# Zhangwenyao1/DreamVLA

Hardware: AMD Instinct MI355X
Metric: train samples/sec (CALVIN ABC->D, seq_len=7) (higher is better)
Workload: dtype bf16; 1 GPU; DreamVLA CALVIN finetune step, head set C (obs_pred+depth_pred+sam_feat_pred+use_dit_head), B=32/GPU, S=7, window 10, 2x224^2 views, 77 text tokens, hidden 1024 / 24 layers / 16 heads, dropout 0.1 on, AdamW + clip 0.1; global_batch=32, seq_len=7, parallelism=dp1, grad_exchange=GradBucketReducer (flat bf16 buckets, async all-reduce), optimizer=FlatAdamW (HIP: dvla_sumsq_bf16 + dvla_adamw_bf16 on flat buffers)

## Files before the change

dreamvla_amd/_lib.py:

```python
import ctypes as C
import os

_HERE = os.path.dirname(os.path.abspath(__file__))
LIB_PATH = os.environ.get("DVLA_LIB") or os.path.join(_HERE, "libdvla_hip.so")

DT_BF16, DT_F32 = 0, 1
CROP_OUT_U8, CROP_OUT_BF16 = 0, 1
ABI_VERSION = 8
ACT = {"none": 0, "gelu": 1, "gelu_erf": 1, "gelu_tanh": 2, "gelu_new": 2, "relu": 3, "silu": 4,
       "quick_gelu": 5, "tanh": 6, "sigmoid": 7}

DVLA_ERRORS = {-1: "invalid argument", -2: "kernel launch failed", -3: "unsupported shape/alignment"}


class DvlaError(RuntimeError):
    pass


class GemmParams(C.Structure):
    _fields_ = [
        ("A", C.c_void_p), ("lda", C.c_int64), ("a_trans", C.c_int32),
        ("B", C.c_void_p), ("ldb", C.c_int64), ("b_trans", C.c_int32),
        ("C", C.c_void_p), ("ldc", C.c_int64), ("c_dtype", C.c_int32),
        ("M", C.c_int64), ("N", C.c_int64), ("K", C.c_int64),
        ("bias", C.c_void_p), ("bias_dtype", C.c_int32),
        ("act", C.c_int32),
        ("preact", C.c_void_p), ("ld_preact", C.c_int64),
        ("dact_aux", C.c_void_p), ("ld_dact", C.c_int64), ("dact", C.c_int32),
        ("dropout_p", C.c_float), ("seed_lo", C.c_uint32), ("seed_hi", C.c_uint32),
        ("residual", C.c_void_p), ("ld_res", C.c_int64), ("res_rows", C.c_int64),
        ("accumulate", C.c_int32),
        ("split_k", C.c_int32), ("workspace", C.c_void_p),
        ("ksum", C.c_void_p), ("ksum_dtype", C.c_int32), ("ksum_operand", C.c_int32), ("ksum_workspace", C.c_void_p),
        ("a_layernorm", C.c_int32), ("a_ln_eps", C.c_float),
    ]


class AttnParams(C.Structure):
    _fields_ = [
        ("q", C.c_void_p), ("k", C.c_void_p), ("v", C.c_void_p), ("o", C.c_void_p),
        ("q_stride_b", C.c_int64), ("q_stride_t", C.c_int64), ("q_stride_h", C.c_int64),
        ("k_stride_b", C.c_int64), ("k_stride_t", C.c_int64), ("k_stride_h", C.c_int64),
        ("v_stride_b", C.c_int64), ("v_stride_t", C.c_int64), ("v_stride_h", C.c_int64),
        ("o_stride_b", C.c_int64), ("o_stride_t", C.c_int64), ("o_stride_h", C.c_int64),
        ("B", C.c_int32), ("H", C.c_int32), ("Lq", C.c_int32), ("Lk", C.c_int32),
        ("scale", C.c_float),
        ("key_index", C.c_void_p), ("mask_bits_q", C.c_void_p), ("mask_bits_k", C.c_void_p),
        ("tile_map", C.c_void_p),
        ("dropout_p", C.c_float), ("seed_lo", C.c_uint32), ("seed_hi", C.c_uint32),
        ("lse", C.c_void_p),
        ("dout", C.c_void_p), ("do_stride_b", C.c_int64), ("do_stride_t", C.c_int64), ("do_stride_h", C.c_int64),
        ("delta", C.c_void_p),
        ("dq", C.c_void_p), ("dk", C.c_void_p), ("dv", C.c_void_p),
        ("dq_stride_b", C.c_int64), ("dq_stride_t", C.c_int64), ("dq_stride_h", C.c_int64),
        ("dk_stride_b", C.c_int64), ("dk_stride_t", C.c_int64), ("dk_stride_h", C.c_int64),
        ("dv_stride_b", C.c_int64), ("dv_stride_t", C.c_int64), ("dv_stride_h", C.c_int64),
    ]


class MaskRule(C.Structure):
    _fields_ = [("K", C.c_int32), ("num_A", C.c_int32), ("num_B", C.c_int32), ("num_obs", C.c_int32),
                ("action_pred_steps", C.c_int32), ("atten_goal", C.c_int32), ("atten_goal_state", C.c_int32),
                ("atten_only_obs", C.c_int32), ("attn_robot_proprio_state", C.c_int32), ("n_drop", C.c_int32)]


class TokenSrc(C.Structure):
    _fields_ = [("base", C.c_void_p), ("stride_b", C.c_int64), ("stride_s", C.c_int64), ("tok_begin", C.c_int32),
                ("tok_count", C.c_int32)]


class DitSampleParams(C.Structure):
    _fields_ = [("blocks", C.c_void_p),
                ("xemb_w", C.c_void_p), ("xemb_b", C.c_void_p), ("final_w", C.c_void_p), ("final_b", C.c_void_p),
                ("pos", C.c_void_p), ("cond", C.c_void_p),
                ("coef", C.c_void_p), ("noise", C.c_void_p), ("out", C.c_void_p),
                ("workspace", C.c_void_p), ("workspace_bytes", C.c_int64),
                ("cfg_scale", C.c_float), ("ln_eps", C.c_float),
                ("depth", C.c_int32), ("hidden", C.c_int32), ("heads", C.c_int32), ("channels", C.c_int32),
                ("tokens", C.c_int32), ("bs", C.c_int32), ("steps", C.c_int32), ("reserved", C.c_int32)]


class FrameView(C.Structure):
    _fields_ = [("base", C.c_void_p), ("stride_b", C.c_int64), ("stride_t", C.c_int64), ("T", C.c_int32)]


class MaeLossParams(C.Structure):
    _fields_ = [("pred", C.c_void_p), ("pred_stride_n", C.c_int64), ("pred_stride_r", C.c_int64), ("row0", C.c_int32),
                ("patch", C.c_int32),
                ("imgs", C.c_void_p), ("imgs_dtype", C.c_int32), ("norm_pix", C.c_int32), ("H", C.c_int32), ("W", C.c_int32),
                ("mask", C.c_void_p), ("N", C.c_int64)]


_P, _I64, _I32, _F, _U32 = C.c_void_p, C.c_int64, C.c_int32, C.c_float, C.c_uint32
SYMBOLS = {
    "dvla_abi_version": (C.c_int, []),
    "dvla_gemm_bf16": (C.c_int, [C.POINTER(GemmParams), _P]),
    "dvla_gemm_ksum_partial_rows": (C.c_int64, [C.c_int32]),
    "dvla_set_gemm_variant": (None, [C.c_int]),
    "dvla_last_gemm_variant": (C.c_int, []),
    "dvla_set_gemm_schedule": (None, [C.c_int, C.c_int]),
    "dvla_get_gemm_schedule": (None, [C.POINTER(C.c_int), C.POINTER(C.c_int)]),
    "dvla_layernorm_fwd": (C.c_int, [_P, _P, _P, _I32, _P, _P, _P, _I64, _I64, _F, _P]),
    "dvla_layernorm_bwd": (C.c_int, [_P, _P, _P, _I32, _P, _P, _P, _P, _P, _P, _I64, _I64, _P]),
    "dvla_layernorm_bwd_add": (C.c_int, [_P, _P, _P, _I32, _P, _P, _P, _P, _P, _P, _I32, _P, _I64, _I64, _P]),
    "dvla_layernorm_bwd_partial_rows": (_I64, []),
    "dvla_layernorm_fwd_rows": (C.c_int, [_P, _P, _P, _I32, _P, _P, _P, _I64, _I64, _F, _I32, _I32, _I32, _I32, _P]),
    "dvla_layernorm_bwd_rows": (C.c_int, [_P, _P, _P, _I32, _P, _P, _P, _P, _P, _I32, _P, _I64, _I64, _I32, _I32, _I32, _I32, _P]),
    "dvla_attn_fwd": (C.c_int, [C.POINTER(AttnParams), _P]),
    "dvla_attn_bwd": (C.c_int, [C.POINTER(AttnParams), _P]),
    "dvla_attn_small_fwd": (C.c_int, [C.POINTER(AttnParams), _I32, _P]),
    "dvla_attn_small_bwd": (C.c_int, [C.POINTER(AttnParams), _I32, _P]),
    "dvla_attn_hd_fwd": (C.c_int, [C.POINTER(AttnParams), _I32, _P]),
    "dvla_attn_hd_bwd": (C.c_int, [C.POINTER(AttnParams), _I32, _P]),
    "dvla_colsum": (C.c_int, [_P, _I64, _I64, _I64, _P, _P, _P]),
    "dvla_colsum_dt": (C.c_int, [_P, _I64, _I64, _I64, _P, _I32, _P, _P]),
    "dvla_colsum_partial_rows": (_I64, []),
    "dvla_dropout": (C.c_int, [_P, _P, _I64, _I64, _F, _U32, _U32, _P]),
    "dvla_act_bwd": (C.c_int, [_P, _P, _P, _I64, _I64, _I32, _F, _U32, _U32, _P]),
    "dvla_act_bwd_colsum": (C.c_int, [_P, _P, _P, _I64, _I64, _I32, _F, _U32, _U32, _P, _I32, _P, _P]),
    "dvla_act_fwd": (C.c_int, [_P, _P, _I64, _I32, _P]),
    "dvla_ddim_cfg_step": (C.c_int, [_P, _I64, _P, _P, _I64, _I64, _F, _F, _F, _F, _F, _P]),
    "dvla_fm_cfg_step": (C.c_int, [_P, _I64, _P, _P, _I64, _I64, _F, _F, _P]),
    "dvla_dit_sample_workspace_bytes": (C.c_int64, [_I32]),
    "dvla_dit_sample": (C.c_int, [C.POINTER(DitSampleParams), _P]),
    "dvla_dit_sample_fm": (C.c_int, [C.POINTER(DitSampleParams), _P]),
    "dvla_dit_sample_set_stamps": (None, [_P]),
    "dvla_dit_sample_inject_timeouts": (None, [_I32]),
    "dvla_cast_f32_to_bf16": (C.c_int, [_P, _P, _I64, _P]),
    "dvla_cast_bf16_to_f32": (C.c_int, [_P, _P, _I64, _P]),
    "dvla_add": (C.c_int, [_P, _P, _P, _I64, _I64, _P]),
    "dvla_assemble_tokens": (C.c_int, [C.POINTER(TokenSrc), _I32, _P, _I64, _P, _I32, _I32, _I32, _I32, _P]),
    "dvla_mask_tables": (C.c_int, [C.POINTER(MaskRule), _P, _P, _P, _P, _P, _P]),
    "dvla_image_preprocess": (C.c_int, [_P, _P, _P, _I64, _I32, _I32, _I32, C.POINTER(C.c_float), C.POINTER(C.c_float), _P]),
    "dvla_image_resize_u8": (C.c_int, [_P, _P, _I64, _I32, _I32, _I32, _I32, _P, _P, _I32, _P, _P, _I32, _I32, _I32, _I32, _P]),
    "dvla_image_resized_crop": (C.c_int, [_P, _P, _P, _P, _I64, _I32, _I32, _I32, _I32, _I32, _I32, _I32, C.POINTER(C.c_float),
                                          C.POINTER(C.c_float), _P]),
    "dvla_depth_preprocess": (C.c_int, [_P, _P, _P, _I64, _I32, _I32, _I32, _I32, _I32, _I32, _P]),
    "dvla_gather_positions": (C.c_int, [_P, _P, _P, _I32, _I32, _I32, _I32, _I32, _I32, _P]),
    "dvla_dream_render": (C.c_int, [_P, _P, _P, _I64, _I32, _I32, _I32, _I32, C.POINTER(C.c_float), C.POINTER(C.c_float), _P]),
    "dvla_image_quality_partial_len": (C.c_int64, [_I64, _I32, _I32]),
    "dvla_image_quality": (C.c_int, [_P, _P, _I64, _I32, _I32, _P, _P, _P, _P]),
    "dvla_depth_quality_partial_len": (C.c_int64, [_I64, _I32, _I32]),
    "dvla_depth_quality": (C.c_int, [_P, _P, _I64, _I32, _I32, _P, _P, _P, _P]),
    "dvla_loss_partial_len": (C.c_int64, []),
    "dvla_patch_mse_fwd": (C.c_int, [C.POINTER(FrameView), C.POINTER(FrameView), _P, _I64, _P, _P, _P]),
    "dvla_patch_mse_bwd": (C.c_int, [C.POINTER(FrameView), C.POINTER(FrameView), _P, _I64, _P, C.POINTER(FrameView), _P]),
# ... 68 lines not shown
```

dreamvla_amd/csrc/attention.hip:

```cpp
#include "common.h"
#include "../../include/dvla.h"

namespace {

constexpr int AT_THREADS = 256;
constexpr int RM72 = 72;
constexpr int RM_BYTES = 32 * RM72 * 2;
constexpr int PI_BYTES = 16 * 64 * 4;
constexpr float LOG2E = 1.4426950408889634f;
constexpr float LN2 = 0.6931471805599453f;

struct AttnKArgs {
  const bf16_t *q, *k, *v; bf16_t* o;
  int64_t qsb, qst, qsh, ksb, kst, ksh, vsb, vst, vsh, osb, ost, osh;
  int B, H, Lq, Lk;
  float scale;
  const int32_t* key_index;
  const uint32_t *bits_q, *bits_k;
  const uint8_t* tile_map; int nqt, nkt;
  int has_drop; uint32_t drop_thr; float inv_keep; uint32_t seed_lo, seed_hi;
  float c1;
  float* lse;
  const bf16_t* dout; int64_t dsb, dst, dsh;
  float* delta;
// ... 1467 lines not shown
        const float alpha = fast_exp2(m_run - m_safe);
        float rs = 0.f;
#pragma unroll
        for (int rr = 0; rr < 16; ++rr) { sv[rr] = fast_exp2(fmaf(sv[rr], scale_log2, -m_safe)); rs += sv[rr]; }
        rs += __shfl_xor(rs, 32, 64);
        l_run = l_run * alpha + rs;
        m_run = m_new;
        if (__any(alpha != 1.0f)) {
#pragma unroll
          for (int rr = 0; rr < 16; ++rr) { oacc[0][rr] *= alpha; oacc[1][rr] *= alpha; }
        }
        bf16x8 vt4[4];
#pragma unroll
        for (int i = 0; i < 4; ++i) vt4[i] = fa_frag_tr(vs, i >> 1, i & 1, lane);
        __builtin_amdgcn_sched_barrier(0);
        const bf16x8 pf0 = pack_frag(sv), pf1 = pack_frag(sv + 8);
        fa_group4(vt4);
        oacc[0] = __builtin_amdgcn_mfma_f32_32x32x16_bf16(vt4[0], pf0, oacc[0], 0, 0, 0);
        oacc[1] = __builtin_amdgcn_mfma_f32_32x32x16_bf16(vt4[2], pf0, oacc[1], 0, 0, 0);
        oacc[0] = __builtin_amdgcn_mfma_f32_32x32x16_bf16(vt4[1], pf1, oacc[0], 0, 0, 0);
        oacc[1] = __builtin_amdgcn_mfma_f32_32x32x16_bf16(vt4[3], pf1, oacc[1], 0, 0, 0);
      }
      if (q_ok) {
        const float inv_l = l_run > 0.f ? 1.0f / l_run : 0.f;
        store_token(p.o + (int64_t)b * p.osb + (int64_t)q * p.ost + (int64_t)h * p.osh, oacc, inv_l, g, (p.st16 & 1) != 0);
        if (p.lse && g == 0) p.lse[(b * p.H + h) * L + q] = l_run > 0.f ? (m_run + log2f(l_run)) * LN2 : INFINITY;
      }
    }
    __syncthreads();
  }
}


}

static bool attn_span32(int64_t rows, int64_t stride_elems, bool gathered) {
  const int64_t r = gathered ? (rows > (1 << 18) ? rows : (1 << 18)) : rows;
  return stride_elems >= 0 && r * stride_elems * 2 + 128 < (1LL << 32);
}

static bool attn_force_staged() {
  static int v = -1;
  if (v < 0) { const char* e = getenv("DVLA_ATTN_STAGED"); v = (e && e[0] == '1') ? 1 : 0; }
  return v == 1;
}

static bool attn_short_enabled() { const char* e = getenv("DVLA_ATTN_SHORT"); return !(e && e[0] == '0'); }
static bool attn_short_fwd_enabled() { const char* e = getenv("DVLA_ATTN_SHORT_FWD"); return !(e && e[0] == '0'); }
static int attn_num_cus() {
  static int cus = 0;
  if (cus == 0) {
    int dev = 0; hipDeviceProp_t prop;
    cus = (hipGetDevice(&dev) == hipSuccess && hipGetDeviceProperties(&prop, dev) == hipSuccess) ? prop.multiProcessorCount : 256;
  }
  return cus;
}

#ifdef DVLA_ATTN_ABLATION
static int attn_dbg() { const char* e = getenv("DVLA_ATTN_DBG"); return e ? atoi(e) : 0; }
#endif

static dim3 ring_items_grid(int nblk, const AttnKArgs& a) {
  static int forced = -1, cus = 0;
  if (forced < 0) {
    const char* e = getenv("DVLA_ATTN_ITEMS"); forced = e ? atoi(e) : 0;
    int dev = 0; hipDeviceProp_t prop;
// ... 100 lines not shown
  const dim3 grid_dq((unsigned)((a.nqt + 3) / 4), (unsigned)a.H, (unsigned)a.B);
  const dim3 grid_dkv((unsigned)((a.nkt + 3) / 4), (unsigned)a.H, (unsigned)a.B);
  const bool span_kv = attn_span32(a.Lk, a.kst, a.key_index != nullptr) && attn_span32(a.Lk, a.vst, a.key_index != nullptr);
  const bool span_q = attn_span32(a.Lq, a.qst, false) && attn_span32(a.Lq, a.dst, false);
  const bool dq_ring = smem_dq <= 64 * 1024 && span_kv && !attn_force_staged();
  a.fuse_delta = dq_ring ? 1 : 0;
  if (!dq_ring) {
    hipLaunchKernelGGL(attn_delta_kernel, dim3((unsigned)((nrows * 8 + 255) / 256)), dim3(256), 0, stream, a);
    rc = dvla_check_launch();
    if (rc != DVLA_OK) return rc;
  }
  if (dq_ring)
    hipLaunchKernelGGL(attn_bwd_dq_ring_kernel, grid_dq, block, smem_dq, stream, a);
  else
    hipLaunchKernelGGL(attn_bwd_dq_kernel, grid_dq, block, 0, stream, a);
  rc = dvla_check_launch();
  if (rc != DVLA_OK) return rc;
  if (smem_dkv <= 80 * 1024 && span_q && !attn_force_staged()) {
    if (smem_dkv > 64 * 1024) {
      static uint64_t attr_done = 0;
      int dev = 0;
      if (hipGetDevice(&dev) != hipSuccess || dev < 0 || dev >= 64) dev = 0;
      if (!(attr_done & (1ull << dev))) {
        (void)hipFuncSetAttribute(reinterpret_cast<const void*>(attn_bwd_dkv_ring_kernel), hipFuncAttributeMaxDynamicSharedMemorySize, 80 * 1024);
        attr_done |= 1ull << dev;
      }
    }
    hipLaunchKernelGGL(attn_bwd_dkv_ring_kernel, grid_dkv, block, smem_dkv, stream, a);
  }
  else
    hipLaunchKernelGGL(attn_bwd_dkv_kernel, grid_dkv, block, 0, stream, a);
  return dvla_check_launch();
}
```

dreamvla_amd/nn.py:

```python
import torch
from torch import nn

from . import ops


class Linear(nn.Linear):

    def forward(self, x, act="none", residual=None, dropout_p=0.0, ln_eps=None):
        if ln_eps is not None:
            return ops.linear_ln(x, self.weight, self.bias, eps=ln_eps, act=act, residual=residual)
        return ops.linear(x, self.weight, self.bias, act=act, residual=residual, dropout_p=dropout_p)


class LayerNorm(nn.LayerNorm):
    def forward(self, x):
        return ops.layer_norm(x, self.weight, self.bias, self.eps)

    def fork(self, x):
        return ops.layer_norm_fork(x, self.weight, self.bias, self.eps)

    def last_tokens(self, x, keep):
        return ops.layer_norm_last_tokens(x, self.weight, self.bias, self.eps, keep)


# ... 36 lines not shown
        self.head_dim = dim // num_heads
        self.scale = self.head_dim ** -0.5
        self.qkv = Linear(dim, dim * 3, bias=qkv_bias)
        self.proj = Linear(dim, dim)

    def forward(self, x, residual=None, ln_eps=None):
        qkv = self.qkv(x, ln_eps=ln_eps)
        o = ops.self_attention(qkv, self.num_heads, scale=self.scale, head_dim=self.head_dim)
        return self.proj(o, residual=residual)


class Block(nn.Module):

    def __init__(self, dim, num_heads, mlp_ratio=4.0, qkv_bias=False, norm_layer=None, act="gelu_erf"):
        super().__init__()
        norm_layer = norm_layer or LayerNorm
        self.norm1 = norm_layer(dim)
        self.attn = Attention(dim, num_heads=num_heads, qkv_bias=qkv_bias)
        self.norm2 = norm_layer(dim)
        self.mlp = Mlp(in_features=dim, hidden_features=int(dim * mlp_ratio), act=act)

    def forward(self, x):
        if isinstance(self.norm1, LayerNorm) and isinstance(self.norm2, LayerNorm):
            r, n = self.norm1.fork(x)
            x = self.attn(n, residual=r)
            r, n = self.norm2.fork(x)
            return self.mlp(n, residual=r)
        x = self.attn(self.norm1(x), residual=x)
        x = self.mlp(self.norm2(x), residual=x)
        return x

    def forward_shared_suffix(self, prefix, suffix, n_seq):
        x = ops.concat_shared_suffix(prefix, suffix)
        qkv = ops.concat_shared_suffix(self.attn.qkv(self.norm1(prefix)), self.attn.qkv(self.norm1(suffix)))
        o = ops.self_attention(qkv, self.attn.num_heads, scale=self.attn.scale, head_dim=self.attn.head_dim)
        x = self.attn.proj(o, residual=x)
        r, n = self.norm2.fork(x)
        return self.mlp(n, residual=r)


class PatchEmbed(nn.Module):

    def __init__(self, img_size=224, patch_size=16, in_chans=3, embed_dim=768):
        super().__init__()
        self.img_size = (img_size, img_size)
        self.patch_size = (patch_size, patch_size)
        self.grid_size = (img_size // patch_size, img_size // patch_size)
        self.num_patches = self.grid_size[0] * self.grid_size[1]
        self.proj = nn.Conv2d(in_chans, embed_dim, kernel_size=patch_size, stride=patch_size)

    def forward(self, x, pos=None):
        n, c, hh, ww = x.shape
        p = self.patch_size[0]
        gh, gw = hh // p, ww // p
        cols = x.view(n, c, gh, p, gw, p).permute(0, 2, 4, 1, 3, 5).reshape(n * gh * gw, c * p * p)
        w = self.proj.weight.view(self.proj.weight.shape[0], -1)
        y = ops.linear(cols, w, self.proj.bias, residual=pos, res_rows=(gh * gw if pos is not None else 0))
        return y.view(n, gh * gw, -1)
```

dreamvla_amd/ops.py:

```python
import ctypes as C
import math
import os

import torch

from . import _lib
from ._lib import ACT, AttnParams, DT_BF16, DT_F32, GemmParams, check

BF16 = torch.bfloat16


def _stream():
    return torch.cuda.current_stream().cuda_stream


def _req(t, name, dtype=BF16):
    if not isinstance(t, torch.Tensor):
        raise TypeError(f"{name}: expected a tensor")
    if not t.is_cuda:
        raise _lib.DvlaError(f"{name}: tensor is on {t.device}; the DreamVLA HIP path has no CPU fallback")
    if dtype is not None and t.dtype != dtype:
        raise TypeError(f"{name}: expected {dtype}, got {t.dtype} (the kernels compute in bf16; fp32 parameters / activations "
                        f"are accepted by the module-level operators -- linear, mlp, layer_norm, attention -- which keep "
                        f"fp32 masters and run on bf16 shadows)")
# ... 1407 lines not shown
    def forward(ctx, prefix, suffix):
        lib = _lib.load()
        _req(prefix, "concat_shared_suffix.prefix"); _req(suffix, "concat_shared_suffix.suffix")
        n, nq, D = prefix.shape
        ns = suffix.shape[0]
        if suffix.shape[1] != D or D % 8 != 0:
            raise ValueError("concat_shared_suffix: (n, nq, D) and (ns, D) with D % 8 == 0")
        if not (prefix.stride(2) == 1 and prefix.stride(1) == D and prefix.stride(0) % 8 == 0 and prefix.data_ptr() % 16 == 0):
            prefix = prefix.contiguous()
        suffix = suffix.contiguous()
        srcs = (_lib.TokenSrc * 2)()
        srcs[0] = _lib.TokenSrc(prefix.data_ptr(), prefix.stride(0), 0, 0, nq)
        srcs[1] = _lib.TokenSrc(suffix.data_ptr(), 0, 0, nq, ns)
        out = torch.empty((n, nq + ns, D), dtype=BF16, device=prefix.device)
        check(lib.dvla_assemble_tokens(srcs, 2, None, D, out.data_ptr(), n, 1, nq + ns, D, _stream()), "dvla_assemble_tokens")
        ctx.nq, ctx.ns = nq, ns
        return out

    @staticmethod
    def backward(ctx, g):
        g = _req(g, "concat_shared_suffix.grad").contiguous()
        n, L, D = g.shape
        dp = g[:, :ctx.nq] if ctx.needs_input_grad[0] else None
        ds = None
        if ctx.needs_input_grad[1]:
            ds = colsum(g.view(n, L * D)[:, ctx.nq * D:], out_dtype=BF16).view(ctx.ns, D)
        return dp, ds


def concat_shared_suffix(prefix, suffix):
    return _ConcatSharedSuffix.apply(to_compute(prefix), to_compute(suffix))


def assemble_tokens(parts, pos=None):
    if len(parts) > 16:
        raise ValueError("assemble_tokens: at most 16 parts")
    return _AssembleTokens.apply(to_compute(pos), *[to_compute(t) for t in parts])


class _Dropout(torch.autograd.Function):
    @staticmethod
    def forward(ctx, x, p):
        _req(x, "dropout.input")
        seed = next_seed()
        ctx.p, ctx.seed, ctx.shape = p, seed, x.shape
        return dropout_raw(x.reshape(-1, x.shape[-1]), p, seed).view(x.shape)

    @staticmethod
    def backward(ctx, dy):
        return dropout_raw(dy.reshape(-1, ctx.shape[-1]), ctx.p, ctx.seed).view(ctx.shape), None


def dropout(x, p, training):
    if not training or p <= 0.0:
        return x
    return _Dropout.apply(to_compute(x), float(p))


class _Act(torch.autograd.Function):
    @staticmethod
    def forward(ctx, x, act):
        _req(x, "act.input")
        ctx.act = act
        if ctx.needs_input_grad[0]:
            ctx.save_for_backward(x)
        return act_fwd_raw(x, act)
# ... 300 lines not shown
```

include/dvla.h:

```cpp
#ifndef DVLA_H_
#define DVLA_H_
#include <stdint.h>
#ifdef __cplusplus
extern "C" {
#endif

#define DVLA_DT_BF16 0
#define DVLA_DT_F32 1

#define DVLA_ACT_NONE 0
#define DVLA_ACT_GELU_ERF 1
#define DVLA_ACT_GELU_TANH 2
#define DVLA_ACT_RELU 3
#define DVLA_ACT_SILU 4
#define DVLA_ACT_QUICK_GELU 5
#define DVLA_ACT_TANH 6
#define DVLA_ACT_SIGMOID 7

#define DVLA_ABI_VERSION 8
int dvla_abi_version(void);

typedef struct dvla_gemm_params {
  const void* A; int64_t lda; int32_t a_trans;
  const void* B; int64_t ldb; int32_t b_trans;
// ... 31 lines not shown
                            int32_t grp, int32_t gstride, int32_t goff, int32_t map_output, void* stream);
int dvla_layernorm_bwd_rows(const void* dy, const void* x, const void* gamma, int32_t param_dtype,
                            const float* mean, const float* rstd, void* dx, void* dgamma, void* dbeta,
                            int32_t grad_dtype, float* partial, int64_t rows, int64_t cols,
                            int32_t grp, int32_t gstride, int32_t goff, int32_t map_output, void* stream);

typedef struct dvla_attn_params {
  const void* q; const void* k; const void* v; void* o;
  int64_t q_stride_b, q_stride_t, q_stride_h;
  int64_t k_stride_b, k_stride_t, k_stride_h;
  int64_t v_stride_b, v_stride_t, v_stride_h;
  int64_t o_stride_b, o_stride_t, o_stride_h;
  int32_t B, H, Lq, Lk;
  float scale;
  const int32_t* key_index;
  const uint32_t* mask_bits_q;
  const uint32_t* mask_bits_k;
  const uint8_t* tile_map;
  float dropout_p; uint32_t seed_lo; uint32_t seed_hi;
  float* lse;
  const void* dout; int64_t do_stride_b, do_stride_t, do_stride_h;
  float* delta;
  void* dq; void* dk; void* dv;
  int64_t dq_stride_b, dq_stride_t, dq_stride_h;
  int64_t dk_stride_b, dk_stride_t, dk_stride_h;
  int64_t dv_stride_b, dv_stride_t, dv_stride_h;
} dvla_attn_params;
int dvla_attn_fwd(const dvla_attn_params* p, void* stream);
int dvla_attn_bwd(const dvla_attn_params* p, void* stream);
int dvla_attn_small_fwd(const dvla_attn_params* p, int32_t head_dim, void* stream);
int dvla_attn_small_bwd(const dvla_attn_params* p, int32_t head_dim, void* stream);
int dvla_attn_hd_fwd(const dvla_attn_params* p, int32_t head_dim, void* stream);
int dvla_attn_hd_bwd(const dvla_attn_params* p, int32_t head_dim, void* stream);

int dvla_colsum(const void* x, int64_t ld, int64_t rows, int64_t cols, float* out, float* partial, void* stream);
int dvla_colsum_dt(const void* x, int64_t ld, int64_t rows, int64_t cols, void* out, int32_t out_dtype, float* partial,
                   void* stream);
int64_t dvla_colsum_partial_rows(void);
int dvla_dropout(const void* x, void* y, int64_t rows, int64_t cols, float p, uint32_t seed_lo, uint32_t seed_hi,
                 void* stream);
int dvla_act_bwd(const void* dy, const void* preact, void* dz, int64_t rows, int64_t cols, int32_t act,
                 float dropout_p, uint32_t seed_lo, uint32_t seed_hi, void* stream);
int dvla_act_bwd_colsum(const void* dy, const void* preact, void* dz, int64_t rows, int64_t cols, int32_t act, float dropout_p,
                        uint32_t seed_lo, uint32_t seed_hi, void* colsum, int32_t colsum_dtype, float* partial, void* stream);
int dvla_act_fwd(const void* x, void* y, int64_t n, int32_t act, void* stream);
int dvla_ddim_cfg_step(const void* model_out, int64_t sample_stride, const float* x, float* x_next, int64_t bs, int64_t per_sample,
                       float cfg_scale, float a, float b, float sqrt_acp_prev, float sqrt_1m_acp_prev, void* stream);
int dvla_fm_cfg_step(const void* model_out, int64_t sample_stride, const float* x, float* x_next, int64_t bs, int64_t per_sample,
                     float cfg_scale, float delta, void* stream);
typedef struct dvla_dit_block_weights {
  const void *qkv_w, *qkv_b, *proj_w, *proj_b, *fc1_w, *fc1_b, *fc2_w, *fc2_b;
} dvla_dit_block_weights;
typedef struct dvla_dit_sample_params {
  const dvla_dit_block_weights* blocks;
  const void *xemb_w, *xemb_b, *final_w, *final_b, *pos, *cond;
  const float* coef;
  const float* noise;
  float* out;
  void* workspace;
  int64_t workspace_bytes;
  float cfg_scale, ln_eps;
  int32_t depth, hidden, heads, channels, tokens, bs, steps, reserved;
} dvla_dit_sample_params;
int64_t dvla_dit_sample_workspace_bytes(int32_t hidden);
int dvla_dit_sample(const dvla_dit_sample_params* p, void* stream);
int dvla_dit_sample_fm(const dvla_dit_sample_params* p, void* stream);
// ... 90 lines not shown
```

Measured before the change: 225.2 samples/s.

## Add shared-suffix attention kernels reading prefix and suffix qkv directly

Adds new HIP forward and backward attention kernels that read Q/K/V from a per-sample prefix buffer and a batch-shared suffix buffer, so the concatenated qkv tensor no longer has to be built. The block's shared-suffix forward path now routes through these kernels and falls back to the old concat-plus-attention path on unsupported shapes. Suffix gradients are reduced with a column sum over the batch. The aim is to remove the concat copy and its memory traffic, including on repeated suffix tile loads. The cost is extra kernel complexity and some branching in the tile loaders.

```diff
diff --git a/dreamvla_amd/_lib.py b/dreamvla_amd/_lib.py
--- a/dreamvla_amd/_lib.py
+++ b/dreamvla_amd/_lib.py
@@ -10,6 +10,7 @@
 ACT = {"none": 0, "gelu": 1, "gelu_erf": 1, "gelu_tanh": 2, "gelu_new": 2, "relu": 3, "silu": 4,
        "quick_gelu": 5, "tanh": 6, "sigmoid": 7}
 
+ERR_UNSUPPORTED = -3
 DVLA_ERRORS = {-1: "invalid argument", -2: "kernel launch failed", -3: "unsupported shape/alignment"}
 
 
@@ -55,6 +56,23 @@
         ("dq_stride_b", C.c_int64), ("dq_stride_t", C.c_int64), ("dq_stride_h", C.c_int64),
         ("dk_stride_b", C.c_int64), ("dk_stride_t", C.c_int64), ("dk_stride_h", C.c_int64),
         ("dv_stride_b", C.c_int64), ("dv_stride_t", C.c_int64), ("dv_stride_h", C.c_int64),
+    ]
+
+
+class AttnSuffixParams(C.Structure):
+    _fields_ = [
+        ("prefix", C.c_void_p), ("suffix", C.c_void_p), ("o", C.c_void_p),
+        ("prefix_stride_b", C.c_int64), ("prefix_stride_t", C.c_int64), ("suffix_stride_t", C.c_int64),
+        ("part_stride", C.c_int64), ("head_stride", C.c_int64),
+        ("o_stride_b", C.c_int64), ("o_stride_t", C.c_int64), ("o_stride_h", C.c_int64),
+        ("B", C.c_int32), ("H", C.c_int32), ("Lq", C.c_int32), ("Lk", C.c_int32), ("nq", C.c_int32), ("head_dim", C.c_int32),
+        ("scale", C.c_float),
+        ("dropout_p", C.c_float),
+        ("key_index", C.c_void_p), ("mask_bits_q", C.c_void_p), ("mask_bits_k", C.c_void_p), ("tile_map", C.c_void_p),
+        ("lse", C.c_void_p),
+        ("dout", C.c_void_p), ("do_stride_b", C.c_int64), ("do_stride_t", C.c_int64), ("do_stride_h", C.c_int64),
+        ("dq", C.c_void_p), ("dk", C.c_void_p), ("dv", C.c_void_p),
+        ("dg_stride_b", C.c_int64), ("dg_stride_t", C.c_int64), ("dg_stride_h", C.c_int64),
     ]
 
 
@@ -112,6 +130,8 @@
     "dvla_attn_small_bwd": (C.c_int, [C.POINTER(AttnParams), _I32, _P]),
     "dvla_attn_hd_fwd": (C.c_int, [C.POINTER(AttnParams), _I32, _P]),
     "dvla_attn_hd_bwd": (C.c_int, [C.POINTER(AttnParams), _I32, _P]),
+    "dvla_attn_suffix_fwd": (C.c_int, [C.POINTER(AttnSuffixParams), _P]),
+    "dvla_attn_suffix_bwd": (C.c_int, [C.POINTER(AttnSuffixParams), _P]),
     "dvla_colsum": (C.c_int, [_P, _I64, _I64, _I64, _P, _P, _P]),
     "dvla_colsum_dt": (C.c_int, [_P, _I64, _I64, _I64, _P, _I32, _P, _P]),
     "dvla_colsum_partial_rows": (_I64, []),
diff --git a/dreamvla_amd/csrc/attention.hip b/dreamvla_amd/csrc/attention.hip
--- a/dreamvla_amd/csrc/attention.hip
+++ b/dreamvla_amd/csrc/attention.hip
@@ -1523,6 +1523,357 @@
 }
 
 
+struct SfxSrc {
+  const bf16_t *pre, *suf;
+  int64_t psb;
+  uint32_t pst2, sst2;
+  int cs, hs;
+  int nq;
+};
+
+__global__ __launch_bounds__(SB_THREADS) __attribute__((amdgpu_waves_per_eu(4, 4))) void attn_suffix_fwd_kernel(AttnKArgs p, SfxSrc s) {
+  extern __shared__ __attribute__((aligned(16))) char smem[];
+  const int t = threadIdx.x, lane = t & 63, l31 = lane & 31, g = lane >> 5;
+  const int wave = __builtin_amdgcn_readfirstlane(t >> 6);
+  const int L = p.Lq;
+  const int nt = p.nqt;
+  const int nq = s.nq;
+  const int rounds = (nt + SB_WAVES - 1) / SB_WAVES;
+  const float scale_log2 = p.scale * LOG2E;
+  const uint32_t smem_base = (uint32_t)(uintptr_t)(__attribute__((address_space(3))) char*)smem;
+  const int rl = 8 * (wave & 3) + (lane >> 3);
+  const int oct = (lane & 7) ^ fa_sw(rl);
+  const int t_keep = (gridDim.x % (unsigned)p.H == 0u) ? (nq + 31) >> 5 : nt;
+  auto issue_op = [&](const bf16_t* pre, const bf16_t* suf, uint32_t region, int t_end) {
+    for (int tt = wave >> 2; tt < t_end; tt += 2) {
+      int row = tt * 32 + rl;
+      row = row < L ? row : L - 1;
+      const uint32_t dst = __builtin_amdgcn_readfirstlane(smem_base + region + (uint32_t)(tt * FA_TILE + (wave & 3) * 1024));
+      if (row < nq) fa_glds16(pre, (uint32_t)row * s.pst2 + (uint32_t)(oct * 16), dst);
+      else fa_glds16(suf, (uint32_t)(row - nq) * s.sst2 + (uint32_t)(oct * 16), dst);
+    }
+  };
+  const int n_items = p.B * p.H;
+  int t_end = nt;
+  for (int item = blockIdx.x; item < n_items; item += gridDim.x) {
+    const int b = item / p.H, h = item - b * p.H;
+    const bf16_t* pb = s.pre + (int64_t)b * s.psb + (int64_t)h * s.hs;
+    const bf16_t* sb = s.suf + (int64_t)h * s.hs;
+    issue_op(pb + s.cs, sb + s.cs, 0u, t_end);
+    issue_op(pb + 2 * s.cs, sb + 2 * s.cs, (uint32_t)(nt * FA_TILE), t_end);
+    t_end = t_keep;
+    for (int r = 0; r < rounds; ++r) {
+      const int j = wave + SB_WAVES * r;
+      const bool active = j < nt;
+      const int q = j * 32 + l31;
+      const bool q_ok = active && q < L;
+      const bf16_t* qrow = q < nq ? pb + (int64_t)q * (s.pst2 >> 1) : sb + (int64_t)(q - nq) * (s.sst2 >> 1);
+      bf16x8 qf[4];
+#pragma unroll
+      for (int sl = 0; sl < 4; ++sl) {
+        const uint4 u = load16(qrow + 16 * sl + 8 * g, q_ok);
+        qf[sl] = *reinterpret_cast<const bf16x8*>(&u);
+      }
+      if (r == 0) {
+        fa_wait_vmcnt<0>();
+        __syncthreads();
+      }
+      if (!active) continue;
+      float m_run = -INFINITY, l_run = 0.f;
+      f32x16 oacc[2] = {zero16(), zero16()};
+      for (int kt = 0; kt < nt; ++kt) {
+        const char* ks = smem + (size_t)kt * FA_TILE;
+        const char* vs = smem + (size_t)(nt + kt) * FA_TILE;
+        f32x16 sacc = zero16();
+        {
+          bf16x8 fk[4];
+#pragma unroll
+          for (int sl = 0; sl < 4; ++sl) fk[sl] = fa_frag_rm(ks, l31, sl, g);
+          fa_group4(fk);
+#pragma unroll
+          for (int sl = 0; sl < 4; ++sl) sacc = __builtin_amdgcn_mfma_f32_32x32x16_bf16(fk[sl], qf[sl], sacc, 0, 0, 0);
+        }
+        const int k0 = kt * 32;
+        float sv[16];
+#pragma unroll
+        for (int rr = 0; rr < 16; ++rr) sv[rr] = sacc[rr];
+        if (k0 + 32 > L) {
+          asm volatile("");
+          const uint32_t vg = low_mask(L - k0) >> (4 * g);
+          vis_select16<NEG_INF_BITS>(vg, sv);
+        }
+        float mt = sv[0];
+#pragma unroll
+        for (int rr = 1; rr < 16; ++rr) mt = fmaxf(mt, sv[rr]);
+        mt = fmaxf(mt, __shfl_xor(mt, 32, 64));
+        const float m_new = fmaxf(m_run, ceilf(mt * scale_log2));
+        const float m_safe = (m_new == -INFINITY) ? 0.f : m_new;
+        const float alpha = fast_exp2(m_run - m_safe);
+        float rs = 0.f;
+#pragma unroll
+        for (int rr = 0; rr < 16; ++rr) { sv[rr] = fast_exp2(fmaf(sv[rr], scale_log2, -m_safe)); rs += sv[rr]; }
+        rs += __shfl_xor(rs, 32, 64);
+        l_run = l_run * alpha + rs;
+        m_run = m_new;
+        if (__any(alpha != 1.0f)) {
+#pragma unroll
+          for (int rr = 0; rr < 16; ++rr) { oacc[0][rr] *= alpha; oacc[1][rr] *= alpha; }
+        }
+        bf16x8 vt4[4];
+#pragma unroll
+        for (int i = 0; i < 4; ++i) vt4[i] = fa_frag_tr(vs, i >> 1, i & 1, lane);
+        __builtin_amdgcn_sched_barrier(0);
+        const bf16x8 pf0 = pack_frag(sv), pf1 = pack_frag(sv + 8);
+        fa_group4(vt4);
+        oacc[0] = __builtin_amdgcn_mfma_f32_32x32x16_bf16(vt4[0], pf0, oacc[0], 0, 0, 0);
+        oacc[1] = __builtin_amdgcn_mfma_f32_32x32x16_bf16(vt4[2], pf0, oacc[1], 0, 0, 0);
+        oacc[0] = __builtin_amdgcn_mfma_f32_32x32x16_bf16(vt4[1], pf1, oacc[0], 0, 0, 0);
+        oacc[1] = __builtin_amdgcn_mfma_f32_32x32x16_bf16(vt4[3], pf1, oacc[1], 0, 0, 0);
+      }
+      if (q_ok) {
+        const float inv_l = l_run > 0.f ? 1.0f / l_run : 0.f;
+        store_token(p.o + (int64_t)b * p.osb + (int64_t)q * p.ost + (int64_t)h * p.osh, oacc, inv_l, g, (p.st16 & 1) != 0);
+        if (p.lse && g == 0) p.lse[(b * p.H + h) * L + q] = l_run > 0.f ? (m_run + log2f(l_run)) * LN2 : INFINITY;
+      }
+    }
+    __syncthreads();
+  }
+}
+
+__global__ __launch_bounds__(SB_THREADS) void attn_suffix_bwd_kernel(AttnKArgs p, SfxSrc s) {
+  extern __shared__ __attribute__((aligned(16))) char smem[];
+  const int t = threadIdx.x, lane = t & 63, l31 = lane & 31, g = lane >> 5;
+  const int wave = __builtin_amdgcn_readfirstlane(t >> 6);
+  const int L = p.Lq;
+  const int nt = p.nqt;
+  const int nq = s.nq;
+  const int rounds = (nt + SB_WAVES - 1) / SB_WAVES;
+  const float scale_log2 = p.scale * LOG2E;
+
+  char* const regA = smem;
+  char* const regB = smem + (size_t)2 * nt * FA_TILE;
+  float* const lse2s = reinterpret_cast<float*>(smem + (size_t)4 * nt * FA_TILE);
+  float* const dlts = lse2s + 32 * nt;
+  const uint32_t smem_base = (uint32_t)(uintptr_t)(__attribute__((address_space(3))) char*)smem;
+  const uint32_t offA = 0u, offB = (uint32_t)(2 * nt * FA_TILE);
+
+  const int rl = 8 * (wave & 3) + (lane >> 3);
+  const int oct = (lane & 7) ^ fa_sw(rl);
+  const int t_keep = (gridDim.x % (unsigned)p.H == 0u) ? (nq + 31) >> 5 : nt;
+  auto issue_src_tile = [&](const bf16_t* pre, const bf16_t* suf, uint32_t region, int tt) {
+    int row = tt * 32 + rl;
+    row = row < L ? row : L - 1;
+    const uint32_t dst = __builtin_amdgcn_readfirstlane(smem_base + region + (uint32_t)(tt * FA_TILE + (wave & 3) * 1024));
+    if (row < nq) fa_glds16(pre, (uint32_t)row * s.pst2 + (uint32_t)(oct * 16), dst);
+    else fa_glds16(suf, (uint32_t)(row - nq) * s.sst2 + (uint32_t)(oct * 16), dst);
+  };
+  const uint32_t dst2 = (uint32_t)p.dst * 2u;
+  auto issue_do_tile = [&](const bf16_t* base, int tt) {
+    int row = tt * 32 + rl;
+    row = row < L ? row : L - 1;
+    const uint32_t dst = smem_base + offA + (uint32_t)((nt + tt) * FA_TILE + (wave & 3) * 1024);
+    fa_glds16(base, (uint32_t)row * dst2 + (uint32_t)(oct * 16), __builtin_amdgcn_readfirstlane(dst));
+  };
+  auto issue_A_tile = [&](int item, int tt, int t_end) {
+    const int b = item / p.H, h = item - b * p.H;
+    if (tt < t_end) issue_src_tile(s.pre + (int64_t)b * s.psb + (int64_t)h * s.hs, s.suf + (int64_t)h * s.hs, offA, tt);
+    issue_do_tile(p.dout + (int64_t)b * p.dsb + (int64_t)h * p.dsh, tt);
+  };
+  auto issue_B = [&](int item, int t_end) {
+    const int b = item / p.H, h = item - b * p.H;
+    const bf16_t* pb = s.pre + (int64_t)b * s.psb + (int64_t)h * s.hs;
+    const bf16_t* sb = s.suf + (int64_t)h * s.hs;
+    for (int tt = wave >> 2; tt < t_end; tt += 2) {
+      issue_src_tile(pb + s.cs, sb + s.cs, offB, tt);
+      issue_src_tile(pb + 2 * s.cs, sb + 2 * s.cs, offB + (uint32_t)(nt * FA_TILE), tt);
+    }
+  };
+
+  const int n_items = p.B * p.H;
+  int item = blockIdx.x;
+  if (item >= n_items) return;
+  for (int tt = wave >> 2; tt < nt; tt += 2) issue_A_tile(item, tt, nt);
+  issue_B(item, nt);
+
+  uint4 ofr[4];
+  float lse_in = 0.f;
+  auto prefetch_o = [&](int it_) {
+    const int b_ = it_ / p.H, h_ = it_ - b_ * p.H;
+    const bf16_t* ob_ = p.o + (int64_t)b_ * p.osb + (int64_t)h_ * p.osh;
+    const int q = wave * 32 + l31;
+    const bool ok = wave < nt && q < L;
+#pragma unroll
+    for (int sl = 0; sl < 4; ++sl) ofr[sl] = load16(ob_ + (int64_t)q * p.ost + 16 * sl + 8 * g, ok);
+    lse_in = ok ? p.lse[(b_ * p.H + h_) * L + q] : 0.f;
+  };
+  prefetch_o(item);
+
+  for (; item < n_items; item += gridDim.x) {
+    const int b = item / p.H, h = item - b * p.H;
+    const int next = item + (int)gridDim.x;
+    const int row0 = (b * p.H + h) * L;
+    const bf16_t* ob = p.o + (int64_t)b * p.osb + (int64_t)h * p.osh;
+
+    fa_wait_vmcnt<0>();
+#pragma unroll
+    for (int sl = 0; sl < 4; ++sl) { fa_settle(ofr[sl].x); fa_settle(ofr[sl].y); fa_settle(ofr[sl].z); fa_settle(ofr[sl].w); }
+    fa_settle(lse_in);
+    __syncthreads();
+
+    for (int r = 0; r < rounds; ++r) {
+      const int j = wave + SB_WAVES * r;
+      if (j >= nt) break;
+      const int q = j * 32 + l31;
+      const bool q_ok = q < L;
+      if (r > 0) {
+#pragma unroll
+        for (int sl = 0; sl < 4; ++sl) ofr[sl] = load16(ob + (int64_t)q * p.ost + 16 * sl + 8 * g, q_ok);
+        lse_in = q_ok ? p.lse[row0 + q] : 0.f;
+      }
+      const char* qs = regA + (size_t)j * FA_TILE;
+      const char* dos = regA + (size_t)(nt + j) * FA_TILE;
+      bf16x8 qf[4], dof[4];
+#pragma unroll
+      for (int sl = 0; sl < 4; ++sl) { qf[sl] = fa_frag_rm(qs, l31, sl, g); dof[sl] = fa_frag_rm(dos, l31, sl, g); }
+      float acc = 0.f;
+#pragma unroll
+      for (int sl = 0; sl < 4; ++sl) {
+        const uint4 dv = *reinterpret_cast<const uint4*>(&dof[sl]);
+        const uint32_t ow[4] = {ofr[sl].x, ofr[sl].y, ofr[sl].z, ofr[sl].w}, dw[4] = {dv.x, dv.y, dv.z, dv.w};
+#pragma unroll
+        for (int i = 0; i < 4; ++i) {
+          acc += bf2f((bf16_t)(dw[i] & 0xffff)) * bf2f((bf16_t)(ow[i] & 0xffff));
+          acc += bf2f((bf16_t)(dw[i] >> 16)) * bf2f((bf16_t)(ow[i] >> 16));
+        }
+      }
+      acc += __shfl_xor(acc, 32, 64);
+      const float lse2 = q_ok ? lse_in * LOG2E : INFINITY;
+      const float dlt = q_ok ? acc * p.scale : 0.f;
+      if (g == 0) { lse2s[j * 32 + l31] = lse2; dlts[j * 32 + l31] = dlt; }
+      f32x16 dqacc[2] = {zero16(), zero16()};
+      for (int kt = 0; kt < nt; ++kt) {
+        const char* ks = regB + (size_t)kt * FA_TILE;
+        const char* vs = regB + (size_t)(nt + kt) * FA_TILE;
+        f32x16 sacc = zero16(), dpacc = zero16();
+        {
+          bf16x8 fk[4], fv[4];
+#pragma unroll
+          for (int sl = 0; sl < 4; ++sl) { fk[sl] = fa_frag_rm(ks, l31, sl, g); fv[sl] = fa_frag_rm(vs, l31, sl, g); }
+          fa_group4(fk); fa_group4(fv);
+#pragma unroll
+          for (int sl = 0; sl < 4; ++sl) {
+            sacc = __builtin_amdgcn_mfma_f32_32x32x16_bf16(fk[sl], qf[sl], sacc, 0, 0, 0);
+            dpacc = __builtin_amdgcn_mfma_f32_32x32x16_bf16(fv[sl], dof[sl], dpacc, 0, 0, 0);
+          }
+        }
+        const int k0 = kt * 32;
+        float ds[16];
+#pragma unroll
+        for (int rr = 0; rr < 16; ++rr) ds[rr] = fast_exp2(fmaf(sacc[rr], scale_log2, -lse2));
+        if (k0 + 32 > L) {
+          asm volatile("");
+          const uint32_t vg = low_mask(L - k0) >> (4 * g);
+          vis_select16<0u>(vg, ds);
+        }
+#pragma unroll
+        for (int rr = 0; rr < 16; ++rr) ds[rr] = ds[rr] * fmaf(dpacc[rr], p.scale, -dlt);
+        const bf16x8 f0 = pack_frag(ds), f1 = pack_frag(ds + 8);
+        bf16x8 kt4[4];
+#pragma unroll
+        for (int i = 0; i < 4; ++i) kt4[i] = fa_frag_tr(ks, i >> 1, i & 1, lane);
+        fa_group4(kt4);
+        dqacc[0] = __builtin_amdgcn_mfma_f32_32x32x16_bf16(kt4[0], f0, dqacc[0], 0, 0, 0);
+        dqacc[1] = __builtin_amdgcn_mfma_f32_32x32x16_bf16(kt4[2], f0, dqacc[1], 0, 0, 0);
+        dqacc[0] = __builtin_amdgcn_mfma_f32_32x32x16_bf16(kt4[1], f1, dqacc[0], 0, 0, 0);
+        dqacc[1] = __builtin_amdgcn_mfma_f32_32x32x16_bf16(kt4[3], f1, dqacc[1], 0, 0, 0);
+      }
+      if (q_ok) store_token(p.dq + (int64_t)b * p.dqsb + (int64_t)q * p.dqst + (int64_t)h * p.dqsh, dqacc, 1.0f, g, (p.st16 & 2) != 0);
+    }
+    __syncthreads();
+
+    for (int r = 0; r < rounds; ++r) {
+      const int j = wave + SB_WAVES * r;
+      const bool active = j < nt;
+      const int key = j * 32 + l31;
+      const bool key_ok = active && key < L;
+      bf16x8 kf[4], vf[4];
+      if (active) {
+        const char* ks = regB + (size_t)j * FA_TILE;
+        const char* vs = regB + (size_t)(nt + j) * FA_TILE;
+#pragma unroll
+        for (int sl = 0; sl < 4; ++sl) { kf[sl] = fa_frag_rm(ks, l31, sl, g); vf[sl] = fa_frag_rm(vs, l31, sl, g); }
+      }
+      if (r == rounds - 1) {
+        __syncthreads();
+        if (next < n_items) { prefetch_o(next); issue_B(next, t_keep); }
+      }
+      const bool last_round = r == rounds - 1;
+      if (!active && !last_round) continue;
+      f32x16 dkacc[2] = {zero16(), zero16()}, dvacc[2] = {zero16(), zero16()};
+      for (int qt = 0; qt < nt; ++qt) {
+        const char* qs = regA + (size_t)qt * FA_TILE;
+        const char* dos = regA + (size_t)(nt + qt) * FA_TILE;
+        if (qt > 0 && last_round) {
+          __syncthreads();
+          if (next < n_items && (wave >> 2) == ((qt - 1) & 1)) issue_A_tile(next, qt - 1, t_keep);
+        }
+        if (!active) continue;
+        f32x16 sacc = zero16(), dpacc = zero16();
+        {
+          bf16x8 fq[4], fd[4];
+#pragma unroll
+          for (int sl = 0; sl < 4; ++sl) { fq[sl] = fa_frag_rm(qs, l31, sl, g); fd[sl] = fa_frag_rm(dos, l31, sl, g); }
+          fa_group4(fq); fa_group4(fd);
+#pragma unroll
+          for (int sl = 0; sl < 4; ++sl) {
+            sacc = __builtin_amdgcn_mfma_f32_32x32x16_bf16(fq[sl], kf[sl], sacc, 0, 0, 0);
+            dpacc = __builtin_amdgcn_mfma_f32_32x32x16_bf16(fd[sl], vf[sl], dpacc, 0, 0, 0);
+          }
+        }
+        const int q0 = qt * 32;
+        float pr[16], ds[16];
+#pragma unroll
+        for (int rq = 0; rq < 4; ++rq) {
+          const float4 a = *reinterpret_cast<const float4*>(lse2s + q0 + 8 * rq + 4 * g);
+          const float4 c = *reinterpret_cast<const float4*>(dlts + q0 + 8 * rq + 4 * g);
+          const float l4[4] = {a.x, a.y, a.z, a.w}, d4[4] = {c.x, c.y, c.z, c.w};
+#pragma unroll
+          for (int e = 0; e < 4; ++e) {
+            const int rr = 4 * rq + e;
+            float pv = fast_exp2(fmaf(sacc[rr], scale_log2, -l4[e]));
+            pv = key_ok ? pv : 0.f;
+            pr[rr] = pv;
+            ds[rr] = pv * fmaf(dpacc[rr], p.scale, -d4[e]);
+          }
+        }
+        const bf16x8 pf0 = pack_frag(pr), pf1 = pack_frag(pr + 8);
+        const bf16x8 sf0 = pack_frag(ds), sf1 = pack_frag(ds + 8);
+        {
+          bf16x8 td[4], tq[4];
+#pragma unroll
+          for (int i = 0; i < 4; ++i) { td[i] = fa_frag_tr(dos, i >> 1, i & 1, lane); tq[i] = fa_frag_tr(qs, i >> 1, i & 1, lane); }
+          fa_group4(td); fa_group4(tq);
+          dvacc[0] = __builtin_amdgcn_mfma_f32_32x32x16_bf16(td[0], pf0, dvacc[0], 0, 0, 0);
+          dkacc[0] = __builtin_amdgcn_mfma_f32_32x32x16_bf16(tq[0], sf0, dkacc[0], 0, 0, 0);
+          dvacc[1] = __builtin_amdgcn_mfma_f32_32x32x16_bf16(td[2], pf0, dvacc[1], 0, 0, 0);
+          dkacc[1] = __builtin_amdgcn_mfma_f32_32x32x16_bf16(tq[2], sf0, dkacc[1], 0, 0, 0);
+          dvacc[0] = __builtin_amdgcn_mfma_f32_32x32x16_bf16(td[1], pf1, dvacc[0], 0, 0, 0);
+          dkacc[0] = __builtin_amdgcn_mfma_f32_32x32x16_bf16(tq[1], sf1, dkacc[0], 0, 0, 0);
+          dvacc[1] = __builtin_amdgcn_mfma_f32_32x32x16_bf16(td[3], pf1, dvacc[1], 0, 0, 0);
+          dkacc[1] = __builtin_amdgcn_mfma_f32_32x32x16_bf16(tq[3], sf1, dkacc[1], 0, 0, 0);
+        }
+      }
+      if (key_ok) {
+        store_token(p.dk + (int64_t)b * p.dksb + (int64_t)key * p.dkst + (int64_t)h * p.dksh, dkacc, 1.0f, g, (p.st16 & 4) != 0);
+        store_token(p.dv + (int64_t)b * p.dvsb + (int64_t)key * p.dvst + (int64_t)h * p.dvsh, dvacc, 1.0f, g, (p.st16 & 8) != 0);
+      }
+    }
+    __syncthreads();
+    if (next < n_items && (wave >> 2) == ((nt - 1) & 1)) issue_A_tile(next, nt - 1, t_keep);
+  }
+}
+
+
 }
 
 static bool attn_span32(int64_t rows, int64_t stride_elems, bool gathered) {
@@ -1689,3 +2040,95 @@
     hipLaunchKernelGGL(attn_bwd_dkv_kernel, grid_dkv, block, 0, stream, a);
   return dvla_check_launch();
 }
+
+static int fill_suffix_args(const dvla_attn_suffix_params* q, bool bwd, AttnKArgs& a, SfxSrc& s) {
+  if (!q || !q->prefix || !q->suffix || !q->o) return DVLA_ERR_ARG;
+  if (q->B <= 0 || q->H <= 0 || q->Lq <= 0 || q->Lk <= 0 || q->nq <= 0) return DVLA_ERR_ARG;
+  if (q->dropout_p < 0.f || q->dropout_p >= 1.f || !(q->scale > 0.f)) return DVLA_ERR_ARG;
+  if (q->key_index || q->mask_bits_q || q->mask_bits_k || q->tile_map || q->dropout_p > 0.f || q->head_dim != 64 || q->Lq != q->Lk)
+    return DVLA_ERR_UNSUPPORTED;
+  if (q->nq >= q->Lk) return DVLA_ERR_ARG;
+  const int nt = (q->Lq + 31) / 32;
+  if (nt > SB_MAX_TILES || attn_force_staged()) return DVLA_ERR_UNSUPPORTED;
+  if ((int64_t)q->B * q->H * q->Lq >= (1LL << 31)) return DVLA_ERR_UNSUPPORTED;
+  if (q->prefix_stride_b < 0 || q->prefix_stride_t <= 0 || q->suffix_stride_t <= 0 || q->part_stride <= 0 || q->head_stride <= 0 ||
+      q->part_stride >= (1LL << 30) || q->head_stride >= (1LL << 30))
+    return DVLA_ERR_UNSUPPORTED;
+  if (!ok16(q->prefix, q->prefix_stride_b, q->prefix_stride_t, q->part_stride) || !ok16(q->suffix, q->suffix_stride_t, q->part_stride, q->head_stride))
+    return DVLA_ERR_UNSUPPORTED;
+  if (!attn_span32(q->nq, q->prefix_stride_t, false) || !attn_span32(q->Lk - q->nq, q->suffix_stride_t, false)) return DVLA_ERR_UNSUPPORTED;
+  if (!(reinterpret_cast<uintptr_t>(q->o) % 8 == 0 && q->o_stride_b % 4 == 0 && q->o_stride_t % 4 == 0 && q->o_stride_h % 4 == 0))
+    return DVLA_ERR_UNSUPPORTED;
+  a = AttnKArgs{};
+  a.o = (bf16_t*)q->o; a.osb = q->o_stride_b; a.ost = q->o_stride_t; a.osh = q->o_stride_h;
+  a.B = q->B; a.H = q->H; a.Lq = q->Lq; a.Lk = q->Lk;
+  a.scale = q->scale; a.inv_keep = 1.0f; a.c1 = q->scale;
+  a.nqt = nt; a.nkt = nt;
+  a.lse = q->lse;
+  a.st16 = ok16(q->o, q->o_stride_b, q->o_stride_t, q->o_stride_h) ? 1 : 0;
+  s.pre = (const bf16_t*)q->prefix; s.suf = (const bf16_t*)q->suffix;
+  s.psb = q->prefix_stride_b;
+  s.pst2 = (uint32_t)(q->prefix_stride_t * 2); s.sst2 = (uint32_t)(q->suffix_stride_t * 2);
+  s.cs = (int)q->part_stride; s.hs = (int)q->head_stride;
+  s.nq = q->nq;
+  if (!bwd) return DVLA_OK;
+  if (!q->dout || !q->lse || !q->dq || !q->dk || !q->dv) return DVLA_ERR_ARG;
+  if (!ok16(q->dout, q->do_stride_b, q->do_stride_t, q->do_stride_h) || !ok16(q->o, q->o_stride_b, q->o_stride_t, q->o_stride_h) ||
+      !attn_span32(q->Lq, q->do_stride_t, false))
+    return DVLA_ERR_UNSUPPORTED;
+  auto ok8 = [&](const void* ptr) {
+    return (reinterpret_cast<uintptr_t>(ptr) % 8 == 0) && (q->dg_stride_b % 4 == 0) && (q->dg_stride_t % 4 == 0) && (q->dg_stride_h % 4 == 0);
+  };
+  if (!ok8(q->dq) || !ok8(q->dk) || !ok8(q->dv)) return DVLA_ERR_UNSUPPORTED;
+  a.dout = (const bf16_t*)q->dout; a.dsb = q->do_stride_b; a.dst = q->do_stride_t; a.dsh = q->do_stride_h;
+  a.dq = (bf16_t*)q->dq; a.dk = (bf16_t*)q->dk; a.dv = (bf16_t*)q->dv;
+  a.dqsb = a.dksb = a.dvsb = q->dg_stride_b; a.dqst = a.dkst = a.dvst = q->dg_stride_t; a.dqsh = a.dksh = a.dvsh = q->dg_stride_h;
+  const bool g16 = q->dg_stride_b % 8 == 0 && q->dg_stride_t % 8 == 0 && q->dg_stride_h % 8 == 0;
+  auto p16 = [&](const void* ptr) { return g16 && reinterpret_cast<uintptr_t>(ptr) % 16 == 0; };
+  a.st16 |= (p16(q->dq) ? 2 : 0) | (p16(q->dk) ? 4 : 0) | (p16(q->dv) ? 8 : 0);
+  return DVLA_OK;
+}
+
+static unsigned suffix_grid(int64_t resident, int64_t items, int H) {
+  int64_t wgs = resident < items ? resident : items;
+  if (wgs >= H) wgs -= wgs % H;
+  return (unsigned)wgs;
+}
+
+extern "C" int dvla_attn_suffix_fwd(const dvla_attn_suffix_params* q, void* stream_) {
+  hipStream_t stream = reinterpret_cast<hipStream_t>(stream_);
+  AttnKArgs a; SfxSrc s;
+  int rc = fill_suffix_args(q, false, a, s);
+  if (rc != DVLA_OK) return rc;
+  static uint64_t attr_done = 0;
+  int dev = 0;
+  if (hipGetDevice(&dev) != hipSuccess || dev < 0 || dev >= 64) dev = 0;
+  if (!(attr_done & (1ull << dev))) {
+    (void)hipFuncSetAttribute(reinterpret_cast<const void*>(attn_suffix_fwd_kernel), hipFuncAttributeMaxDynamicSharedMemorySize, 80 * 1024);
+    attr_done |= 1ull << dev;
+  }
+  const unsigned wgs = suffix_grid((int64_t)attn_num_cus() * 2, (int64_t)a.B * a.H, a.H);
+  hipLaunchKernelGGL(attn_suffix_fwd_kernel, dim3(wgs), dim3(SB_THREADS), sf_smem_bytes(a.nqt), stream, a, s);
+  return dvla_check_launch();
+}
+
+extern "C" int dvla_attn_suffix_bwd(const dvla_attn_suffix_params* q, void* stream_) {
+  hipStream_t stream = reinterpret_cast<hipStream_t>(stream_);
+  AttnKArgs a; SfxSrc s;
+  int rc = fill_suffix_args(q, true, a, s);
+  if (rc != DVLA_OK) return rc;
+  const size_t smem = sb_smem_bytes(a.nqt);
+  static uint64_t attr_done = 0;
+  int dev = 0;
+  if (hipGetDevice(&dev) != hipSuccess || dev < 0 || dev >= 64) dev = 0;
+  if (!(attr_done & (1ull << dev))) {
+    (void)hipFuncSetAttribute(reinterpret_cast<const void*>(attn_suffix_bwd_kernel), hipFuncAttributeMaxDynamicSharedMemorySize, 160 * 1024);
+    attr_done |= 1ull << dev;
+  }
+  int per_cu = (int)((size_t)(160 * 1024) / smem);
+  if (per_cu < 1) per_cu = 1;
+  if (per_cu > 2048 / SB_THREADS) per_cu = 2048 / SB_THREADS;
+  const unsigned wgs = suffix_grid((int64_t)attn_num_cus() * per_cu, (int64_t)a.B * a.H, a.H);
+  hipLaunchKernelGGL(attn_suffix_bwd_kernel, dim3(wgs), dim3(SB_THREADS), smem, stream, a, s);
+  return dvla_check_launch();
+}
diff --git a/dreamvla_amd/nn.py b/dreamvla_amd/nn.py
--- a/dreamvla_amd/nn.py
+++ b/dreamvla_amd/nn.py
@@ -92,8 +92,8 @@
 
     def forward_shared_suffix(self, prefix, suffix, n_seq):
         x = ops.concat_shared_suffix(prefix, suffix)
-        qkv = ops.concat_shared_suffix(self.attn.qkv(self.norm1(prefix)), self.attn.qkv(self.norm1(suffix)))
-        o = ops.self_attention(qkv, self.attn.num_heads, scale=self.attn.scale, head_dim=self.attn.head_dim)
+        o = ops.self_attention_shared_suffix(self.attn.qkv(self.norm1(prefix)), self.attn.qkv(self.norm1(suffix)),
+                                             self.attn.num_heads, self.attn.scale, head_dim=self.attn.head_dim)
         x = self.attn.proj(o, residual=x)
         r, n = self.norm2.fork(x)
         return self.mlp(n, residual=r)
diff --git a/dreamvla_amd/ops.py b/dreamvla_amd/ops.py
--- a/dreamvla_amd/ops.py
+++ b/dreamvla_amd/ops.py
@@ -1463,6 +1463,83 @@
     return _ConcatSharedSuffix.apply(to_compute(prefix), to_compute(suffix))
 
 
+class _SuffixAttentionUnsupported(Exception):
+    """dvla_attn_suffix_fwd declined the shape (DVLA_ERR_UNSUPPORTED): the caller materialises the qkv buffer instead"""
+
+
+def _attn_suffix_params(prefix, suffix, o, lse, H, scale):
+    n, nq, W = prefix.shape
+    ns = suffix.shape[0]
+    D = W // (3 * H)
+    p = _lib.AttnSuffixParams()
+    p.prefix, p.suffix, p.o = prefix.data_ptr(), suffix.data_ptr(), o.data_ptr()
+    p.prefix_stride_b, p.prefix_stride_t, p.suffix_stride_t = prefix.stride(0), prefix.stride(1), suffix.stride(0)
+    p.part_stride, p.head_stride = H * D, D
+    p.o_stride_b, p.o_stride_t, p.o_stride_h = o.stride(0), o.stride(1), o.stride(2)
+    p.B, p.H, p.Lq, p.Lk, p.nq, p.head_dim = n, H, nq + ns, nq + ns, nq, D
+    p.scale = float(scale)
+    p.lse = _ptr(lse)
+    return p
+
+
+class _SelfAttentionSharedSuffix(torch.autograd.Function):
+
+    @staticmethod
+    def forward(ctx, prefix, suffix, H, scale):
+        lib = _lib.load()
+        _req(prefix, "self_attention_shared_suffix.prefix"); _req(suffix, "self_attention_shared_suffix.suffix")
+        n, nq, W = prefix.shape
+        ns = suffix.shape[0]
+        prefix, suffix = prefix.contiguous(), suffix.contiguous()
+        need_grad = any(ctx.needs_input_grad)
+        o = torch.empty((n, nq + ns, H, 64), dtype=BF16, device=prefix.device)
+        lse = torch.empty((n, H, nq + ns), dtype=torch.float32, device=prefix.device) if need_grad else None
+        p = _attn_suffix_params(prefix, suffix, o, lse, H, scale)
+        rc = lib.dvla_attn_suffix_fwd(C.byref(p), _stream())
+        if rc == _lib.ERR_UNSUPPORTED:
+            raise _SuffixAttentionUnsupported()
+        check(rc, "dvla_attn_suffix_fwd")
+        ctx.H, ctx.scale = H, scale
+        if need_grad:
+            ctx.save_for_backward(prefix, suffix, o, lse)
+        return o.view(n, nq + ns, W // 3)
+
+    @staticmethod
+    def backward(ctx, dout):
+        lib = _lib.load()
+        prefix, suffix, o, lse = ctx.saved_tensors
+        n, nq, W = prefix.shape
+        ns, H = suffix.shape[0], ctx.H
+        L = nq + ns
+        dqkv = torch.empty((n, L, W), dtype=BF16, device=prefix.device)
+        d5 = dqkv.view(n, L, 3, H, 64)
+        do = _req(dout, "attention.grad_output").contiguous().view(n, L, H, 64)
+        p = _attn_suffix_params(prefix, suffix, o, lse, H, ctx.scale)
+        p.dout = do.data_ptr()
+        p.do_stride_b, p.do_stride_t, p.do_stride_h = do.stride(0), do.stride(1), do.stride(2)
+        p.dq, p.dk, p.dv = d5[:, :, 0].data_ptr(), d5[:, :, 1].data_ptr(), d5[:, :, 2].data_ptr()
+        p.dg_stride_b, p.dg_stride_t, p.dg_stride_h = d5.stride(0), d5.stride(1), d5.stride(3)
+        check(lib.dvla_attn_suffix_bwd(C.byref(p), _stream()), "dvla_attn_suffix_bwd")
+        dp = dqkv[:, :nq] if ctx.needs_input_grad[0] else None
+        ds = None
+        if ctx.needs_input_grad[1]:
+            ds = colsum(dqkv.view(n, L * W)[:, nq * W:], out_dtype=BF16).view(ns, W)
+        return dp, ds, None, None
+
+
+def self_attention_shared_suffix(qkv_prefix, qkv_suffix, num_heads, scale=None, *, mask_tables=None, dropout_p=0.0, head_dim=64):
+    scale = (1.0 / math.sqrt(float(head_dim))) if scale is None else scale
+    qkv_prefix, qkv_suffix = to_compute(qkv_prefix), to_compute(qkv_suffix)
+    if (head_dim == 64 and mask_tables is None and dropout_p == 0.0 and qkv_prefix.dim() == 3 and qkv_suffix.dim() == 2
+            and qkv_prefix.shape[2] == qkv_suffix.shape[1] == 3 * num_heads * 64):
+        try:
+            return _SelfAttentionSharedSuffix.apply(qkv_prefix, qkv_suffix, int(num_heads), float(scale))
+        except _SuffixAttentionUnsupported:
+            pass
+    return self_attention(concat_shared_suffix(qkv_prefix, qkv_suffix), num_heads, scale=scale, mask_tables=mask_tables,
+                          dropout_p=dropout_p, head_dim=head_dim)
+
+
 def assemble_tokens(parts, pos=None):
     if len(parts) > 16:
         raise ValueError("assemble_tokens: at most 16 parts")
diff --git a/include/dvla.h b/include/dvla.h
--- a/include/dvla.h
+++ b/include/dvla.h
@@ -87,6 +87,25 @@
 int dvla_attn_small_bwd(const dvla_attn_params* p, int32_t head_dim, void* stream);
 int dvla_attn_hd_fwd(const dvla_attn_params* p, int32_t head_dim, void* stream);
 int dvla_attn_hd_bwd(const dvla_attn_params* p, int32_t head_dim, void* stream);
+typedef struct dvla_attn_suffix_params {
+  const void* prefix; const void* suffix; void* o;
+  int64_t prefix_stride_b, prefix_stride_t, suffix_stride_t;
+  int64_t part_stride, head_stride;
+  int64_t o_stride_b, o_stride_t, o_stride_h;
+  int32_t B, H, Lq, Lk, nq, head_dim;
+  float scale;
+  float dropout_p;
+  const int32_t* key_index;
+  const uint32_t* mask_bits_q;
+  const uint32_t* mask_bits_k;
+  const uint8_t* tile_map;
+  float* lse;
+  const void* dout; int64_t do_stride_b, do_stride_t, do_stride_h;
+  void* dq; void* dk; void* dv;
+  int64_t dg_stride_b, dg_stride_t, dg_stride_h;
+} dvla_attn_suffix_params;
+int dvla_attn_suffix_fwd(const dvla_attn_suffix_params* p, void* stream);
+int dvla_attn_suffix_bwd(const dvla_attn_suffix_params* p, void* stream);
 
 int dvla_colsum(const void* x, int64_t ld, int64_t rows, int64_t cols, float* out, float* partial, void* stream);
 int dvla_colsum_dt(const void* x, int64_t ld, int64_t rows, int64_t cols, void* out, int32_t out_dtype, float* partial,
```

Measured after the change: 226.4 samples/s (median of 4 runs). Within noise of the previous version (+0.5%).
